# thetisproject/thetis

Hardware: AMD Instinct MI355X
Metric: DG element-updates/sec, 2D SWE DG-P1 SSPRK33 (higher is better)
Workload: dtype f64

## Files before the change

thetis_amd/csrc/swe2d_api_fuse.hip:

```cpp
#include "swe2d_handle.h"
#include "swe2d_fuse.h"
#include "swe2d_tiles.h"

#include <type_traits>

namespace swe2d_impl {

namespace {
template <bool... B, class F> auto pick_instance(F f) { return f(std::bool_constant<B>{}...); }
template <bool... B, class F, class... Rest> auto pick_instance(F f, bool b, Rest... rest)
{
    return b ? pick_instance<B..., true>(f, rest...) : pick_instance<B..., false>(f, rest...);
}

const TileSpec kPairTiles{3, 1, SWE_FUSE_WG, SWE_FUSE_INNER, SWE_FUSE_RING, SWE_FUSE_MAX_OUT, false};
const TileSpec kQuadPairTiles{4, 1, SWE_FUSE_WG, SWE_QFUSE_INNER, SWE_QFUSE_RING, SWE_QFUSE_MAX_OUT, false};
const TileSpec kTripleTiles{3, 2, SWE_FUSE_WG, SWE_FUSE_WG, -1, SWE_FUSE3_MAX_OUT, true, true};

int build_table(Handle *h, const TileSpec &spec, const std::vector<int> &order, const std::vector<unsigned char> &start, TileTable &t)
{
    const int n = h->n_cells;
    std::string err;
    if (build_tiles(h->h_nbr.data(), h->stride, n, (int)order.size() == n ? order.data() : nullptr,
                    (int)start.size() == n ? start.data() : nullptr, spec, t, err))
        return fail(h, SWE2D_ERR_UNSUPPORTED, err);
    return SWE2D_OK;
}

std::vector<int> tile_records(const TileTable &t, int nfacets)
{
    std::vector<int> rec;
    for (size_t i = 0; i < t.cell.size(); i++) {
        const unsigned *w = &t.facet[i*nfacets];
        rec.push_back(t.cell[i]);
        rec.push_back((int)(w[0] | (w[1] << SWE_FUSE_FBITS) | (w[2] << (2*SWE_FUSE_FBITS))));
        if (nfacets == 4) { rec.push_back((int)w[3]); rec.push_back(0); }
    }
    return rec;
}

int upload_tiles(Handle *h, TileSet &ts, const std::vector<int> &rec, const std::vector<int> &counts, const TileTable &t,
                 const std::vector<unsigned> *slot_data = nullptr)
{
    HIP_TRY(h, hipMalloc(&ts.tile, rec.size()*sizeof(int)));
    HIP_TRY(h, hipMalloc(&ts.counts, counts.size()*sizeof(int)));
    HIP_TRY(h, hipMemcpy(ts.tile, rec.data(), rec.size()*sizeof(int), hipMemcpyHostToDevice));
    HIP_TRY(h, hipMemcpy(ts.counts, counts.data(), counts.size()*sizeof(int), hipMemcpyHostToDevice));
    std::vector<int> slots;
    for (size_t i = 0; i + 1 < t.slot_first.size(); i++) { slots.push_back(t.slot_first[i]); slots.push_back(t.slot_first[i + 1] - t.slot_first[i]); }
    std::vector<int> src(t.slot_src);
    if (slot_data) src.assign(slot_data->begin(), slot_data->end());
    src.push_back(0);
    HIP_TRY(h, hipMalloc(&ts.slots, slots.size()*sizeof(int)));
    HIP_TRY(h, hipMalloc(&ts.slot_src, src.size()*sizeof(int)));
    HIP_TRY(h, hipMemcpy(ts.slots, slots.data(), slots.size()*sizeof(int), hipMemcpyHostToDevice));
    HIP_TRY(h, hipMemcpy(ts.slot_src, src.data(), src.size()*sizeof(int), hipMemcpyHostToDevice));
    ts.n_tiles = (int)t.n_inner.size();
    ts.ring[0] = t.ring[0]; ts.ring[1] = t.ring[1];
    return SWE2D_OK;
}
}

void free_tiles(TileSet &ts)
{
    if (ts.tile) (void)hipFree(ts.tile);
    if (ts.counts) (void)hipFree(ts.counts);
    if (ts.slots) (void)hipFree(ts.slots);
    if (ts.slot_src) (void)hipFree(ts.slot_src);
    ts = TileSet();
}

int fuse12_build(Handle *h)
{
    TileSet &ts = pair_tiles(h);
    if (ts.tile || h->fuse_state == -1 || stream_capturing(h)) return SWE2D_OK;
    TileTable t;
    if (int rc = build_table(h, h->npc == 4 ? kQuadPairTiles : kPairTiles, h->fuse_order, {}, t)) return rc;
    if (!fuse12_tiles_pay(h, (int)t.n_inner.size())) { h->fuse_state = -1; return SWE2D_OK; }
    return upload_tiles(h, ts, tile_records(t, h->npc), t.n_inner, t);
}

template <class Args>
static int launch_pair(Handle *h, void (*kern)(const Args), int cell_end)
{
    const TileSet &ts = pair_tiles(h);
    if (!ts.tile) return fail(h, SWE2D_ERR_UNSUPPORTED, "fused stage pair: no tile tables");
    Args q;
    fill_stage_args(h, q.st, 0, 0, 2, 0.0, 1.0, kBeta[0], 0, h->n_owned);
    q.st.idxc = h->opt[SWE2D_OPT_COMPACT_IDX] == 0 ? nullptr : h->idxc;
    q.tile = static_cast<decltype(q.tile)>(ts.tile);
    q.n_inner = ts.counts;
    q.n_tiles = ts.n_tiles;
    q.cell_end = cell_end;
    q.beta1 = kBeta[0];
    q.a0_2 = kAlpha0[1]; q.a1_2 = kAlphaIn[1]; q.beta2 = kBeta[1];
    q.out = h->state[2];
    const int grid = ((ts.n_tiles + 7)/8)*8;
    SWE_CHK_SYNC(h->stream);
    hipLaunchKernelGGL(kern, dim3(grid), dim3(SWE_FUSE_WG), 0, h->stream, q);
    HIP_TRY(h, hipGetLastError());
    stage_written(h, false, true);
    return SWE2D_OK;
}

int launch_fuse12(Handle *h, int cell_end)
{
    const bool nl = h->par.use_nonlinear_equations != 0, lf = h->par.use_lax_friedrichs_velocity != 0;
    if (h->npc == 4)
        return launch_pair(h, pick_instance([](auto a, auto b, auto c, auto d) -> void (*)(const SweFuseQuadArgs) {
                               return swe_fuse12_quad_kernel<a.value, b.value, c.value, d.value>; }, nl, lf, has_sources(h), h->affine), cell_end);
    return launch_pair(h, pick_instance([](auto a, auto b, auto c) -> void (*)(const SweFuseArgs) {
                           return swe_fuse12_kernel<a.value, b.value, c.value>; }, nl, lf, has_sources(h)), cell_end);
}

int fuse123_build(Handle *h)
{
    if (h->fuse3.tile || stream_capturing(h)) return SWE2D_OK;
    TileTable t;
    if (int rc = build_table(h, kTripleTiles, (int)h->fuse3_order.size() == h->n_cells ? h->fuse3_order : h->fuse_order, h->fuse3_start, t)) return rc;
    std::vector<int> counts;
    for (size_t i = 0; i < t.n_inner.size(); i++) { counts.push_back(t.n_inner[i]); counts.push_back(t.n_mid[i] | (t.rot[i] << 16)); }
    LaneRecords r;
    build_lane_records(t, h->h_nbr.data(), h->h_cv.data(), h->stride, SWE_FUSE_WG, 8u*SWE_FUSE3_XG, (unsigned)h->stride*8u, r);
    return upload_tiles(h, h->fuse3, r.lane, counts, t, &r.slot);
}

int launch_fuse123(Handle *h, int cell_end)
{
    if (int rc = capture_parity_check(h)) return rc;
    if (int rc = fuse123_build(h)) return rc;
    if (!h->fuse3.tile) return fail(h, SWE2D_ERR_UNSUPPORTED, "fused stages: no tile tables (not built inside a stream capture)");
    SweFuse3Args q;
    fill_stage_args(h, q.st, 0, 0, 1, 0.0, 1.0, kBeta[0], 0, h->n_owned);
    q.rec = static_cast<const int4 *>(h->fuse3.tile);
    q.counts = reinterpret_cast<const int2 *>(h->fuse3.counts);
    q.slots = reinterpret_cast<const int2 *>(h->fuse3.slots);
    q.slot_off = reinterpret_cast<const uint2 *>(h->fuse3.slot_src);
    q.n_tiles = h->fuse3.n_tiles;
    q.cell_end = cell_end;
    for (int s = 0; s < 3; s++) { q.a0[s] = s ? kAlpha0[s] : 0.0; q.a1[s] = s ? kAlphaIn[s] : 1.0; q.beta[s] = kBeta[s]; }
    q.out = h->state[1];
    auto kern = pick_instance([](auto a, auto b, auto c) -> void (*)(const SweFuse3Args) { return swe_fuse123_kernel<a.value, b.value, c.value>; },
                              h->par.use_nonlinear_equations != 0, h->par.use_lax_friedrichs_velocity != 0, has_sources(h));
    const int grid = ((h->fuse3.n_tiles + 7)/8)*8;
    SWE_CHK_SYNC(h->stream);
    hipLaunchKernelGGL(kern, dim3(grid), dim3(SWE_FUSE_WG), 0, h->stream, q);
    HIP_TRY(h, hipGetLastError());
    swap_state_buffers(h);
    unsigned long long id = 0;
    if (stream_capturing(h, &id)) {
        if (id != h->capture_id) { h->capture_id = id; h->capture_swaps = 0; }
        h->capture_swaps++;
    }
    return SWE2D_OK;
}

int capture_parity_check(Handle *h)
{
    if (h->capture_swaps == 0 && h->capture_odd == 0) return SWE2D_OK;
    unsigned long long id = 0;
    const bool capturing = stream_capturing(h, &id);
    if (h->capture_swaps) {
        if (capturing && id == h->capture_id) return SWE2D_OK;
        if (h->capture_swaps & 1) { swap_state_buffers(h); h->capture_odd++; }
        h->capture_swaps = 0;
    }
    if (capturing || h->capture_odd == 0) return SWE2D_OK;
    const int odd = h->capture_odd;
    h->capture_odd = 0;
    return fail(h, SWE2D_ERR_UNSUPPORTED, std::to_string(odd) + " stream capture(s) recorded an odd number of swe2d_solve_step_cells launches: "
                "such a graph ends on the other state buffer than it began on and cannot be replayed (the state is the one from before the "
                "capture); capture an even number per sequence");
}

}

static int checked_tile_order(Handle *h, const int32_t *cells, std::vector<int> &order)
{
    std::vector<char> seen((size_t)h->n_cells, 0);
    for (int i = 0; cells && i < h->n_cells; i++) {
        if (cells[i] < 0 || cells[i] >= h->n_cells || seen[cells[i]]) return fail(h, SWE2D_ERR_INVALID_ARGUMENT, "fused stages: the tile order is not a permutation of the cells");
        seen[cells[i]] = 1;
    }
    if (cells) order.assign(cells, cells + h->n_cells);
    return SWE2D_OK;
}

extern "C" {

int swe2d_fused_set_order(swe2d_handle *hh, const int32_t *cells_in_tile_order)
{
    Handle *h = H(hh);
    if (!h) return SWE2D_ERR_INVALID_ARGUMENT;
    HIP_TRY(h, hipSetDevice(h->device));
    std::vector<int> order;
    if (int rc = checked_tile_order(h, cells_in_tile_order, order)) return rc;
    HIP_TRY(h, hipStreamSynchronize(h->stream));
    for (TileSet *ts : {&h->fuse, &h->fuseq, &h->fuse3}) free_tiles(*ts);
    if (h->fuse_state == -1) h->fuse_state = 0;
    h->fuse_order.swap(order);
    return SWE2D_OK;
}

int swe2d_fused_set_triple_tiles(swe2d_handle *hh, const int32_t *cells_in_tile_order, const int32_t *tile_starts, int32_t n_starts)
{
    Handle *h = H(hh);
    if (!h) return SWE2D_ERR_INVALID_ARGUMENT;
    HIP_TRY(h, hipSetDevice(h->device));
    std::vector<int> order;
    std::vector<unsigned char> start;
    if (int rc = checked_tile_order(h, cells_in_tile_order, order)) return rc;
    if (n_starts < 0 || (n_starts > 0 && !tile_starts)) return fail(h, SWE2D_ERR_INVALID_ARGUMENT, "fused stages: tile starts");
    if (n_starts > 0) {
        start.assign((size_t)h->n_cells, 0);
        for (int i = 0; i < n_starts; i++) {
            if (tile_starts[i] < 0 || tile_starts[i] >= h->n_cells) return fail(h, SWE2D_ERR_INVALID_ARGUMENT, "fused stages: a tile start outside the cells");
            start[tile_starts[i]] = 1;
        }
    }
    HIP_TRY(h, hipStreamSynchronize(h->stream));
    free_tiles(h->fuse3);
    h->fuse3_order.swap(order);
    h->fuse3_start.swap(start);
    return SWE2D_OK;
}

static int fused_triple_info(Handle *h, StepCaller who, int32_t out[4])
{
    if (!h || !out) return fail(h, SWE2D_ERR_INVALID_ARGUMENT, "null argument");
    out[0] = out[1] = out[2] = out[3] = 0;
    HIP_TRY(h, hipSetDevice(h->device));
    StepPath path;
    if (int rc = step_ready(h, who, kTriple, &path)) return rc;
    if (path != kTriple) return SWE2D_OK;
    out[0] = 1; out[1] = h->fuse3.n_tiles; out[2] = (int32_t)h->fuse3.ring[0]; out[3] = (int32_t)h->fuse3.ring[1];
    return SWE2D_OK;
}
int swe2d_fused_triple_info(swe2d_handle *hh, int32_t out[4]) { return fused_triple_info(H(hh), kWholeStep, out); }
int swe2d_fused_step_info(swe2d_handle *hh, int32_t out[4]) { return fused_triple_info(H(hh), kPartitionStep, out); }

int swe2d_solve_step_cells(swe2d_handle *hh, int32_t cell_end)
{
    Handle *h = H(hh);
    if (!h) return SWE2D_ERR_INVALID_ARGUMENT;
    if (cell_end < 0 || cell_end > h->n_cells) return fail(h, SWE2D_ERR_INVALID_ARGUMENT, "bad cell range");
    if (!(step_kernels(h) & kTriple)) return fail(h, SWE2D_ERR_UNSUPPORTED, "swe2d_solve_step_cells: the three-stage kernel does not cover this handle");
    HIP_TRY(h, hipSetDevice(h->device));
    if (int rc = capture_parity_check(h)) return rc;
    if (!h->fuse3.tile && stream_capturing(h))
        return fail(h, SWE2D_ERR_UNSUPPORTED, "swe2d_solve_step_cells: first call inside a stream capture (swe2d_fused_step_info builds the tables)");
    return launch_fuse123(h, cell_end);
}

int swe2d_solve_stage_pair_cells(swe2d_handle *hh, int32_t cell_end_0, int32_t cell_end_1)
{
    Handle *h = H(hh);
    if (!h) return SWE2D_ERR_INVALID_ARGUMENT;
    if (cell_end_1 < 0 || cell_end_1 > cell_end_0 || cell_end_0 > h->n_cells) return fail(h, SWE2D_ERR_INVALID_ARGUMENT, "bad cell ranges");
    if (forced(h)) return fail(h, SWE2D_ERR_UNSUPPORTED, "swe2d_solve_stage_pair_cells: not with a tide table or an atmospheric record (swe2d_tide_eval / swe2d_atm_eval + swe2d_solve_stage_cells per stage)");
    HIP_TRY(h, hipSetDevice(h->device));
    if (int rc = capture_parity_check(h)) return rc;
    StepPath path;
    if (int rc = step_ready(h, kPartitionPair, kPair, &path)) return rc;
    if (path == kPair) return launch_fuse12(h, cell_end_1);
    if (int rc = stage_on_range(h, 0, 0, cell_end_0)) return rc;
    return stage_on_range(h, 1, 0, cell_end_1);
}

}
```

thetis_amd/csrc/swe2d_fuse.h:

```cpp
#pragma once
#include "swe2d_kernels.h"
#include "swe2d_flow.h"

#ifndef SWE_FUSE_WG
#define SWE_FUSE_WG 256
#endif
#ifndef SWE_FUSE_MIN_WG
#define SWE_FUSE_MIN_WG 3
#endif
#ifndef SWE_FUSE_INNER
#define SWE_FUSE_INNER 192
#endif
#define SWE_FUSE_FBITS 10
#define SWE_FUSE_RING (SWE_FUSE_WG - SWE_FUSE_INNER)
#define SWE_FUSE_XG (9*SWE_FUSE_WG)
#define SWE_FUSE_MAX_OUT (2*SWE_FUSE_RING)
#define SWE_FUSE_LDS (SWE_FUSE_XG + 6*SWE_FUSE_MAX_OUT)

struct SweFuseArgs {
    SweStageArgs st;
    const int2 *tile;
    const int *n_inner;
    int n_tiles;
    int cell_end;
// ... 68 lines not shown
            py[i] = swe_ld(rvy, v8, 0);
            h[i] = swe_ld(rvh, v8, 0);
        }
#pragma unroll
        for (int f = 0; f < 3; f++) {
            const int b = (f + 1) % 3;
            nx[f] = py[b] - py[f];
            ny[f] = px[f] - px[b];
        }
#pragma unroll
        for (int i = 0; i < 3; i++) { lds[i*SWE_FUSE_WG + lane] = u[i]; lds[(3 + i)*SWE_FUSE_WG + lane] = v[i]; lds[(6 + i)*SWE_FUSE_WG + lane] = e[i]; }
#pragma unroll
        for (int f = 0; f < 3; f++) {
            if (outside[f]) {
                const unsigned at = ((unsigned)tl.y >> (SWE_FUSE_FBITS*f)) & 0x1ffu;
#pragma unroll
                for (int j = 0; j < 6; j++) lds[SWE_LDSI(SWE_FUSE_XG + 6*at + j, SWE_FUSE_LDS)] = r0[f][j];
            }
        }
    }
    __syncthreads();
    double o1u[3], o1v[3], o1e[3];
    double twoA = 0.0;
    if (real) {
        twoA = fma(nx[0], ny[1], -(ny[0]*nx[1]));
        double bu[3], bv[3], be[3], wu[3], wv[3], we[3];
        double H[3];
        swe_tri_depths<NONLIN, false>(h, e, nullptr, H);
        swe_tri_cell<NONLIN>(p.g, u, v, e, H, nx, ny, bu, bv, be);
        swe_flow_rhs_facets<NONLIN, LF, SRC, 1, false, SWE_FUSE_XG, SWE_FUSE_WG, SWE_FUSE_LDS>(p, k, u, v, e, h, lds, tr, bmarkers, nx, ny, twoA, bu, bv, be);
#pragma unroll
        for (int i = 0; i < 3; i++) { wu[i] = 1.0*u[i]; wv[i] = 1.0*v[i]; we[i] = 1.0*e[i]; }
        swe_tri_finish<NONLIN, LF, false, true>(p, k, q.beta1, twoA, u, v, e, h, nullptr, nullptr, nx, ny, bmarkers, bkind1, bu, bv, be,
                                                wu, wv, we, true, o1u, o1v, o1e);
    }
    __syncthreads();
    if (real) {
#pragma unroll
        for (int i = 0; i < 3; i++) { lds[i*SWE_FUSE_WG + lane] = o1u[i]; lds[(3 + i)*SWE_FUSE_WG + lane] = o1v[i]; lds[(6 + i)*SWE_FUSE_WG + lane] = o1e[i]; }
    }
    const bool act2 = lane < n_inner && k < q.cell_end;
    if (act2) {
#pragma unroll
        for (int i = 0; i < 3; i++) {
            lw[i][lane] = fma(q.a0_2, u[i], q.a1_2*o1u[i]);
            lw[3 + i][lane] = fma(q.a0_2, v[i], q.a1_2*o1v[i]);
            lw[6 + i][lane] = fma(q.a0_2, e[i], q.a1_2*o1e[i]);
        }
    }
    __syncthreads();
    if (act2) {
#pragma unroll
        for (int i = 0; i < 3; i++) asm volatile("" : "+v"(nx[i]), "+v"(ny[i]), "+v"(h[i]));
#pragma unroll
        for (int f = 0; f < 3; f++) asm volatile("" : "+v"(tr[f][0]));
        asm volatile("" : "+v"(bmarkers), "+v"(twoA));
        double bu[3], bv[3], be[3], wu[3], wv[3], we[3], ou[3], ov[3], oe[3];
        double H[3];
        swe_tri_depths<NONLIN, false>(h, o1e, nullptr, H);
        swe_tri_cell<NONLIN>(p.g, o1u, o1v, o1e, H, nx, ny, bu, bv, be);
        swe_flow_rhs_facets<NONLIN, LF, SRC, 1, false, SWE_FUSE_XG, SWE_FUSE_WG, SWE_FUSE_LDS>(p, k, o1u, o1v, o1e, h, lds, tr, bmarkers, nx, ny, twoA, bu, bv, be);
#pragma unroll
        for (int i = 0; i < 3; i++) { wu[i] = lw[i][lane]; wv[i] = lw[3 + i][lane]; we[i] = lw[6 + i][lane]; }
        swe_tri_finish<NONLIN, LF, false, true>(p, k, q.beta2, twoA, o1u, o1v, o1e, h, nullptr, nullptr, nx, ny, bmarkers, bkind1, bu, bv, be,
                                                wu, wv, we, true, ou, ov, oe);
        const swe_rsrc_t gou = swe_rsrc(q.out), gov = swe_rsrc(q.out + 3*S), goe = swe_rsrc(q.out + 6*S);
#pragma unroll
        for (int i = 0; i < 3; i++) {
            swe_st(gou, k8, i*S8, ou[i]);
            swe_st(gov, k8, i*S8, ov[i]);
            swe_st(goe, k8, i*S8, oe[i]);
        }
    }
}

#ifndef SWE_FUSE3_MAX_OUT
#define SWE_FUSE3_MAX_OUT 224
#endif
#ifndef SWE_FUSE3_GEOM
#define SWE_FUSE3_GEOM 1
#endif
#define SWE_FUSE3_NGEO 7
#define SWE_FUSE3_GEO (18*SWE_FUSE_WG)
#define SWE_FUSE3_XG (SWE_FUSE3_GEOM ? 9*SWE_FUSE_WG : 18*SWE_FUSE_WG)
#define SWE_FUSE3_LDS (SWE_FUSE3_GEOM ? SWE_FUSE3_GEO + SWE_FUSE3_NGEO*SWE_FUSE_WG : SWE_FUSE3_XG + 6*SWE_FUSE3_MAX_OUT)
static_assert(6*SWE_FUSE3_MAX_OUT <= 9*SWE_FUSE_WG, "the staging area must fit P1");
#ifndef SWE_FUSE3_SRC_MIN_WG
#define SWE_FUSE3_SRC_MIN_WG 2
#endif

struct SweFuse3Args {
    SweStageArgs st;
    const int4 *rec;
    const int2 *counts;
    const int2 *slots;
    const uint2 *slot_off;
    int n_tiles;
    int cell_end;
    double a0[3], a1[3], beta[3];
    double *out;
};

template <bool NONLIN, bool LF, bool SRC = false>
__global__ __launch_bounds__(SWE_FUSE_WG, SRC ? SWE_FUSE3_SRC_MIN_WG : SWE_FUSE_MIN_WG) void swe_fuse123_kernel(const SweFuse3Args q)
{
#pragma clang fp contract(off)
    __shared__ double lds[SWE_FUSE3_LDS];
    const SweStageArgs &p = q.st;
    const int tile = swe_logical_block(blockIdx.x, gridDim.x);
    if (tile >= q.n_tiles) return;
    const int lane = (int)threadIdx.x;
    const int4 *const rec = q.rec + (size_t)tile*(2*SWE_FUSE_WG) + lane;
    const int4 ra = rec[0];
    const int4 rb = rec[SWE_FUSE_WG];
    const bool real = ra.x >= 0;
    const int k = real ? ra.x : 0;
    const int2 cnt = q.counts[tile];
    const int n_inner = cnt.x, n_mid = cnt.y & 0xffff, rot64 = (cnt.y >> 16) << 6;
    const size_t S = p.stride;
    const unsigned S8 = (unsigned)S*8u, k8 = (unsigned)k*8u;
    double *const P1 = lds + 9*SWE_FUSE_WG;
#ifdef SWE_WAVE_TIMING
    int wt_bodies = __any(real) ? 1 : 0;
#endif
    const int2 sl = q.slots[tile];
    const int slot = ((lane & 63) << 2) | (lane >> 6);
    const bool has_slot = slot < sl.y;
    uint2 so = {0u, 0u};
    if (has_slot) so = q.slot_off[sl.x + slot];

    int bmarkers = rb.w, bkind1 = 0;
    unsigned tr[3][1] = {{(unsigned)ra.y}, {(unsigned)ra.z}, {(unsigned)ra.w}};
    double h[3], nx[3], ny[3], u[3], v[3], e[3];
    double px[3], py[3];
    const swe_rsrc_t gu = swe_rsrc(p.uin), gv = swe_rsrc(p.uin + 3*S), ge = swe_rsrc(p.uin + 6*S);
    if (real) {
        if (bmarkers != 0) {
            const int m1 = (bmarkers & 0xff) ? (bmarkers & 0xff) : ((bmarkers & 0xff00) ? ((bmarkers >> 8) & 0xff) : (bmarkers >> 16));
            bkind1 = m1 < SWE_MAX_MARKERS ? p.bc.kind[m1] : 0;
        }
#pragma unroll
        for (int i = 0; i < 3; i++) {
            u[i] = swe_ld(gu, k8, i*S8);
            v[i] = swe_ld(gv, k8, i*S8);
            e[i] = swe_ld(ge, k8, i*S8);
        }
        const swe_rsrc_t rvx = swe_rsrc(p.vx), rvy = swe_rsrc(p.vy), rvh = swe_rsrc(p.vh);
        const unsigned v8[3] = {(unsigned)rb.x, (unsigned)rb.y, (unsigned)rb.z};
#pragma unroll
        for (int i = 0; i < 3; i++) {
            px[i] = swe_ld(rvx, v8[i], 0);
            py[i] = swe_ld(rvy, v8[i], 0);
            h[i] = swe_ld(rvh, v8[i], 0);
        }
    }
    double r0[6];
    if (has_slot) {
        const unsigned ob = so.x, oa = so.y;
        r0[0] = swe_ld(gu, ob, 0); r0[1] = swe_ld(gv, ob, 0); r0[2] = swe_ld(ge, ob, 0);
        r0[3] = swe_ld(gu, oa, 0); r0[4] = swe_ld(gv, oa, 0); r0[5] = swe_ld(ge, oa, 0);
    }
    if (real) {
#pragma unroll
        for (int f = 0; f < 3; f++) {
            const int b = (f + 1) % 3;
            nx[f] = py[b] - py[f];
            ny[f] = px[f] - px[b];
        }
#pragma unroll
        for (int i = 0; i < 3; i++) { lds[i*SWE_FUSE_WG + lane] = u[i]; lds[(3 + i)*SWE_FUSE_WG + lane] = v[i]; lds[(6 + i)*SWE_FUSE_WG + lane] = e[i]; }
    }
    if (has_slot) {
#pragma unroll
        for (int j = 0; j < 6; j++) lds[SWE_LDSI(SWE_FUSE3_XG + 6*slot + j, SWE_FUSE3_LDS)] = r0[j];
    }
    __syncthreads();
    constexpr int GEOM1 = SWE_FUSE3_GEOM ? SWE_GEOM_KEEP : SWE_GEOM_COMPUTE, GEOM23 = SWE_FUSE3_GEOM ? SWE_GEOM_STORED : SWE_GEOM_COMPUTE;
    double twoA = 0.0;
    double *const G = lds + SWE_FUSE3_GEO + lane;
    if (real) {
        twoA = fma(nx[0], ny[1], -(ny[0]*nx[1]));
        double bu[3], bv[3], be[3], wu[3], wv[3], we[3], ou[3], ov[3], oe[3];
        double H[3];
        swe_tri_depths<NONLIN, false>(h, e, nullptr, H);
        swe_tri_cell<NONLIN>(p.g, u, v, e, H, nx, ny, bu, bv, be);
        swe_flow_rhs_facets<NONLIN, LF, SRC, 1, false, SWE_FUSE3_XG, SWE_FUSE_WG, SWE_FUSE3_LDS, GEOM1, SWE_TR_BYTES, true>(p, k, u, v, e, h, lds, tr, bmarkers, nx, ny, twoA, bu, bv, be,
                                                                                                     nullptr, nullptr, G);
#pragma unroll
        for (int i = 0; i < 3; i++) { wu[i] = 1.0*u[i]; wv[i] = 1.0*v[i]; we[i] = 1.0*e[i]; }
        swe_tri_finish<NONLIN, LF, false, true, GEOM1, SWE_FUSE_WG>(p, k, q.beta[0], twoA, u, v, e, h, nullptr, nullptr, nx, ny, bmarkers, bkind1,
                                                                    bu, bv, be, wu, wv, we, true, ou, ov, oe, G);
#pragma unroll
        for (int i = 0; i < 3; i++) { u[i] = ou[i]; v[i] = ov[i]; e[i] = oe[i]; }
    }
    if (SWE_FUSE3_GEOM) __syncthreads();
    if (real) {
#pragma unroll
        for (int i = 0; i < 3; i++) { P1[i*SWE_FUSE_WG + lane] = u[i]; P1[(3 + i)*SWE_FUSE_WG + lane] = v[i]; P1[(6 + i)*SWE_FUSE_WG + lane] = e[i]; }
    }
    __syncthreads();
#pragma unroll 1
    for (int s = 1; s < 3; s++) {
        const int role = (lane - rot64) & (SWE_FUSE_WG - 1);
        const bool act = role < (s == 1 ? n_mid : n_inner) && (s == 1 || k < q.cell_end);
#ifdef SWE_WAVE_TIMING
        wt_bodies += __any(act) ? 1 : 0;
#endif
        double ou[3], ov[3], oe[3];
        if (act) {
#pragma unroll
            for (int i = 0; i < 3; i++) asm volatile("" : "+v"(nx[i]), "+v"(ny[i]), "+v"(h[i]));
#pragma unroll
            for (int f = 0; f < 3; f++) asm volatile("" : "+v"(tr[f][0]));
            asm volatile("" : "+v"(bmarkers));
            if (SRC || !SWE_FUSE3_GEOM) asm volatile("" : "+v"(twoA));
            double bu[3], bv[3], be[3], wu[3], wv[3], we[3];
            double H[3];
            swe_tri_depths<NONLIN, false>(h, e, nullptr, H);
            swe_tri_cell<NONLIN>(p.g, u, v, e, H, nx, ny, bu, bv, be);
            swe_flow_rhs_facets<NONLIN, LF, SRC, 1, false, SWE_FUSE3_XG, SWE_FUSE_WG, 9*SWE_FUSE_WG, GEOM23, SWE_TR_BYTES_INSIDE, true>(p, k, u, v, e, h, P1, tr, bmarkers, nx, ny, twoA, bu, bv, be,
                                                                                                          nullptr, nullptr, G);
            const double a0 = q.a0[s], a1 = q.a1[s];
#pragma unroll
            for (int i = 0; i < 3; i++) {
                wu[i] = fma(a0, lds[i*SWE_FUSE_WG + lane], a1*u[i]);
                wv[i] = fma(a0, lds[(3 + i)*SWE_FUSE_WG + lane], a1*v[i]);
                we[i] = fma(a0, lds[(6 + i)*SWE_FUSE_WG + lane], a1*e[i]);
            }
            swe_tri_finish<NONLIN, LF, false, true, GEOM23, SWE_FUSE_WG>(p, k, q.beta[s], twoA, u, v, e, h, nullptr, nullptr, nx, ny, bmarkers,
                                                                         bkind1, bu, bv, be, wu, wv, we, true, ou, ov, oe, G);
        }
        if (s == 1) {
            __syncthreads();
            if (act) {
#pragma unroll
                for (int i = 0; i < 3; i++) { P1[i*SWE_FUSE_WG + lane] = ou[i]; P1[(3 + i)*SWE_FUSE_WG + lane] = ov[i]; P1[(6 + i)*SWE_FUSE_WG + lane] = oe[i]; }
#pragma unroll
                for (int i = 0; i < 3; i++) { u[i] = ou[i]; v[i] = ov[i]; e[i] = oe[i]; }
            }
            __syncthreads();
        } else if (act) {
            const swe_rsrc_t gou = swe_rsrc(q.out), gov = swe_rsrc(q.out + 3*S), goe = swe_rsrc(q.out + 6*S);
#pragma unroll
            for (int i = 0; i < 3; i++) {
                swe_st(gou, k8, i*S8, ou[i]);
                swe_st(gov, k8, i*S8, ov[i]);
                swe_st(goe, k8, i*S8, oe[i]);
            }
        }
    }
#ifdef SWE_WAVE_TIMING
    if ((lane & 63) == 0 && 4*blockIdx.x + (lane >> 6) < 6*SWE_WT_MAX) {
        unsigned hw, xcc;
        asm volatile("s_getreg_b32 %0, hwreg(HW_REG_HW_ID)" : "=s"(hw));
        asm volatile("s_getreg_b32 %0, hwreg(HW_REG_XCC_ID)" : "=s"(xcc));
        (&swe_wave_ts[0][0])[4*blockIdx.x + (lane >> 6)] = (unsigned long long)hw | ((unsigned long long)(xcc & 0xf) << 32)
                                                           | ((unsigned long long)wt_bodies << 40) | (1ull << 44);
    }
#endif
}


#define SWE_QFUSE_INNER 192
#define SWE_QFUSE_RING (SWE_FUSE_WG - SWE_QFUSE_INNER)
#define SWE_QFUSE_XG (12*SWE_FUSE_WG)
#define SWE_QFUSE_MAX_OUT (3*SWE_QFUSE_RING)
#define SWE_QFUSE_LDS (SWE_QFUSE_XG + 6*SWE_QFUSE_MAX_OUT)

struct SweFuseQuadArgs {
    SweStageArgs st;
    const int4 *tile;
    const int *n_inner;
    int n_tiles;
    int cell_end;
    double beta1, a0_2, a1_2, beta2;
    double *out;
};

template <bool NONLIN, bool LF, bool SRC, bool AFFINE>
__global__ __launch_bounds__(SWE_FUSE_WG, SWE_FUSE_MIN_WG) void swe_fuse12_quad_kernel(const SweFuseQuadArgs q)
{
#pragma clang fp contract(off)
    __shared__ double lds[SWE_QFUSE_LDS];
    __shared__ double lu0[12*SWE_QFUSE_INNER];
    const SweStageArgs &p = q.st;
    const int tile = swe_logical_block(blockIdx.x, gridDim.x);
    if (tile >= q.n_tiles) return;
    const int lane = (int)threadIdx.x;
    const int4 tl = q.tile[(size_t)tile*SWE_FUSE_WG + lane];
    const bool real = tl.x >= 0;
    const int k = real ? tl.x : 0;
    const int n_inner = q.n_inner[tile];
    const size_t S = p.stride;
    const unsigned S8 = (unsigned)S*8u, k8 = (unsigned)k*8u, S4 = (unsigned)S*4u, k4 = (unsigned)k*4u;

    unsigned tr[4] = {0u, 0u, 0u, 0u}, bmarkers = 0u;
    int nb[4] = {-1, -1, -1, -1}, vid[4] = {0, 0, 0, 0};
    double u[4], v[4], e[4];
    if (real) {
#pragma unroll
        for (int i = 0; i < 4; i++) {
            nb[i] = swe_ldi(swe_rsrc(p.nbr), k4, i*S4);
            vid[i] = swe_ldi(swe_rsrc(p.cv), k4, i*S4);
        }
        const swe_rsrc_t gu = swe_rsrc(p.uin), gv = swe_rsrc(p.uin + 4*S), ge = swe_rsrc(p.uin + 8*S);
#pragma unroll
        for (int i = 0; i < 4; i++) {
            u[i] = swe_ld(gu, k8, i*S8);
            v[i] = swe_ld(gv, k8, i*S8);
            e[i] = swe_ld(ge, k8, i*S8);
        }
        bmarkers = (nb[0] < 0 ? (unsigned)(-nb[0]) : 0u) | (nb[1] < 0 ? (unsigned)(-nb[1]) << 8 : 0u) |
                   (nb[2] < 0 ? (unsigned)(-nb[2]) << 16 : 0u) | (nb[3] < 0 ? (unsigned)(-nb[3]) << 24 : 0u);
        double r0[4][6];
        bool outside[4];
#pragma unroll
        for (int f = 0; f < 4; f++) {
            const int nbf = nb[f];
            const unsigned w = f < 3 ? (((unsigned)tl.y >> (SWE_FUSE_FBITS*f)) & 0x3ffu) : ((unsigned)tl.z & 0x3ffu);
            outside[f] = (w & 0x200u) != 0u;
            const unsigned at = w & 0x1ffu;
            const int f2 = nbf >= 0 ? (nbf & 3) : f, na = (f2 + 1) & 3;
            const unsigned ab = outside[f] ? (unsigned)(SWE_QFUSE_XG + 6*at) : (unsigned)(f2*SWE_FUSE_WG + at);
            const unsigned aa = outside[f] ? (unsigned)(SWE_QFUSE_XG + 6*at + 3) : (unsigned)(na*SWE_FUSE_WG + at);
            tr[f] = ab | (aa << 16);
            const int code = outside[f] ? nbf : ((k << 2) | f);
            const unsigned kn8 = (unsigned)(code >> 2)*8u;
            const int g2 = code & 3, ga = (g2 + 1) & 3;
            const unsigned ob = kn8 + ((g2 & 1) ? S8 : 0u) + ((g2 & 2) ? 2u*S8 : 0u);
            const unsigned oa = kn8 + ((ga & 1) ? S8 : 0u) + ((ga & 2) ? 2u*S8 : 0u);
            r0[f][0] = swe_ld(gu, ob, 0); r0[f][1] = swe_ld(gv, ob, 0); r0[f][2] = swe_ld(ge, ob, 0);
            r0[f][3] = swe_ld(gu, oa, 0); r0[f][4] = swe_ld(gv, oa, 0); r0[f][5] = swe_ld(ge, oa, 0);
        }
#pragma unroll
        for (int i = 0; i < 4; i++) { lds[i*SWE_FUSE_WG + lane] = u[i]; lds[(4 + i)*SWE_FUSE_WG + lane] = v[i]; lds[(8 + i)*SWE_FUSE_WG + lane] = e[i]; }
#pragma unroll
        for (int f = 0; f < 4; f++) {
            if (outside[f]) {
                const unsigned at = (f < 3 ? ((unsigned)tl.y >> (SWE_FUSE_FBITS*f)) : (unsigned)tl.z) & 0x1ffu;
#pragma unroll
// ... 50 lines not shown
```

thetis_amd/csrc/swe2d_handle.h:

```cpp
#pragma once
#include "../../include/swe2d.h"
#include "swe2d_kernels.h"
#include "swe2d_sipg.h"
#include "swe2d_flow.h"
#include "swe2d_p2p.h"

#include <dlfcn.h>
#include <unistd.h>

#include <algorithm>
#include <cmath>
#include <cstdio>
#include <cstdlib>
#include <cstring>
#include <new>
#include <string>
#include <vector>
#include <atomic>
#include <mutex>

static_assert(SWE2D_MAX_MARKERS == SWE_MAX_MARKERS, "marker table size mismatch");
static_assert(SWE2D_MAX_FARMS == SWE_MAX_FARMS && SWE2D_MAX_THRUST_TABLE == SWE_MAX_THRUST_TABLE, "turbine farm table size mismatch");

#ifdef SWE_RANGE_CHECK
#include <map>
#include <mutex>
namespace {
std::mutex g_chk_mutex;
std::map<unsigned long long, unsigned long long> g_chk_allocs;
bool g_chk_dirty = true;
unsigned long long g_chk_launches = 0;
void swe_chk_upload_locked()
{
    static SweChkTable t;
    t.n = 0;
    for (auto &kv : g_chk_allocs) if (t.n < SWE_CHK_MAX) { t.lo[t.n] = kv.first; t.hi[t.n] = kv.second; t.n++; }
    (void)hipDeviceSynchronize();
    (void)hipMemcpyToSymbol(HIP_SYMBOL(swe_chk_tab), &t, sizeof(t));
    g_chk_dirty = false;
}
hipError_t swe_chk_malloc(void **p, size_t n)
{
    const hipError_t e = hipMalloc(p, n);
    if (e == hipSuccess && *p) {
        std::lock_guard<std::mutex> lock(g_chk_mutex);
        const char *st = getenv("THETIS_AMD_RANGE_SELFTEST");
        g_chk_allocs[(unsigned long long)*p] = (unsigned long long)*p + ((st && atoi(st)) ? n/2 : n);
        swe_chk_upload_locked();
    }
    return e;
}
template <class T> hipError_t swe_chk_malloc(T **p, size_t n) { return swe_chk_malloc((void **)p, n); }
hipError_t swe_chk_free(void *p)
{
    { std::lock_guard<std::mutex> lock(g_chk_mutex); g_chk_allocs.erase((unsigned long long)p); g_chk_dirty = true; }
    return hipFree(p);
}
void swe_chk_sync(hipStream_t stream)
{
    std::lock_guard<std::mutex> lock(g_chk_mutex);
    g_chk_launches++;
    if (!g_chk_dirty) return;
    hipStreamCaptureStatus cs = hipStreamCaptureStatusNone;
    if (stream && hipStreamIsCapturing(stream, &cs) == hipSuccess && cs != hipStreamCaptureStatusNone) return;
    swe_chk_upload_locked();
}
}
#define hipMalloc(p, n) swe_chk_malloc(p, n)
#define hipFree(p) swe_chk_free(p)
#define SWE_CHK_SYNC(stream) swe_chk_sync(stream)
extern "C" int swe2d_debug_range_report(unsigned long long out[5])
{
    std::lock_guard<std::mutex> lock(g_chk_mutex);
    (void)hipDeviceSynchronize();
    if (hipMemcpyFromSymbol(out, HIP_SYMBOL(swe_chk_report), 4*sizeof(unsigned long long)) != hipSuccess) return 1;
    out[3] = g_chk_launches;
    out[4] = g_chk_allocs.size();
    return 0;
}
#else
#define SWE_CHK_SYNC(stream) ((void)0)
#endif

namespace swe2d_impl {

extern thread_local std::string g_create_error;

extern const double kBeta[3], kAlpha0[3], kAlphaIn[3];

extern std::atomic<unsigned long long> g_next_uid;

struct TileSet {
    void *tile = nullptr;
    int *counts = nullptr;
    int *slots = nullptr;
    int *slot_src = nullptr;
    int n_tiles = 0;
    long long ring[2] = {0, 0};
};

struct Handle {
    unsigned long long uid = g_next_uid.fetch_add(1ull);
    int device = 0;
    hipStream_t stream = nullptr;
    bool own_stream = false;
    hipStream_t my_stream = nullptr;
    hipStream_t xstream = nullptr;
    int n_cells = 0, n_owned = 0, n_interior = 0, n_vertices = 0;
    int npc = 3;
    bool affine = true;
    bool affine_local = true;
    size_t stride = 0;
    double *state[3] = {nullptr, nullptr, nullptr};
    int *nbr = nullptr, *cv = nullptr;
    struct FacetList { std::vector<int32_t> cells, facets; int *dev = nullptr; };
    FacetList facet_lists[8];
    int facet_list_next = 0;
    int4 *opp4 = nullptr;
    int *bnd_cells = nullptr;
    int n_bnd = 0;
    int opt[SWE2D_OPT_COUNT];
    Handle() { for (int i = 0; i < SWE2D_OPT_COUNT; i++) opt[i] = -1; }
    bool stage_valid[2] = {false, false};
    int capture_swaps = 0;
    unsigned long long capture_id = 0;
    int capture_odd = 0;
    int4 *idx4 = nullptr;
    int2 *idx2 = nullptr;
    int4 *idxc = nullptr;
    TileSet fuse, fuseq, fuse3;
    int fuse_state = 0;
    std::vector<int> fuse_order;
    std::vector<int> fuse3_order;
    std::vector<unsigned char> fuse3_start;
    int n_conn_escapes = 0;
    std::vector<int> h_nbr;
    std::vector<int> h_cv;
    unsigned *flow_flag = nullptr, *flow_status = nullptr;
    int4 *flow_xo4 = nullptr;
    int2 *flow_xo2 = nullptr;
    int2 *flow_xblk = nullptr;
    int *flow_xsrc = nullptr;
    std::vector<int> h_send, h_recv;
    std::vector<int> flow_fpos;
    int2 *flow_xsend = nullptr;
    int *flow_xrecv = nullptr;
    unsigned *flow_xtick = nullptr;
    int flow_push_blocks = 0, flow_recv_blocks = 0;
    bool flow_x_ready = false;
    int *flow_cell = nullptr;
    unsigned flow_parity_bytes = 0;
    void *flow_ex = nullptr;
    size_t flow_ex_bytes = 0;
    int flow_blocks = 0;
    int flow_capacity = -1;
    int flow_max_rim = 0;
    int launch_parity = 0;
    bool flow_used = false;
    double *vx = nullptr, *vy = nullptr, *vh = nullptr;
    double *bc_field[4] = {nullptr, nullptr, nullptr, nullptr};
    double *valpha = nullptr;
    bool wd = false;
    bool state_holds_D = false;
    struct Snapshot { void *data = nullptr; size_t bytes = 0; bool holds_D = false; };
    Snapshot snapshot[SWE2D_SNAPSHOT_SLOTS];
    bool visc = false;
    double *nu_v = nullptr;
    double nu_const = 0.0, sipg_factor = 1.0;
    int visc_grad_div = 0, visc_grad_depth = 1;
    double *field[SWE2D_FIELD_COUNT] = {nullptr, nullptr, nullptr, nullptr, nullptr, nullptr, nullptr, nullptr, nullptr};
    double scalar[SWE2D_SCALAR_COUNT] = {-1.0, -1.0, -1.0, 0.0, -1.0};
    double *stage_uv = nullptr, *stage_eta = nullptr;
    double *partial = nullptr;
    int n_partial_blocks = 0;
    unsigned long long *diag_acc = nullptr;
    int *send_cells = nullptr, *recv_cells = nullptr;
    int n_send = 0, n_recv = 0;
    struct P2p {
        void *zone = nullptr;
// ... 293 lines not shown
```

thetis_amd/csrc/swe2d_tiles.h:

```cpp
#pragma once
#include <algorithm>
#include <cstddef>
#include <string>
#include <utility>
#include <vector>

#ifndef SWE_FUSE3_ROT
#define SWE_FUSE3_ROT(tile) ((int)(((unsigned)(tile)*0x9E3779B1u) >> 30))
#endif

namespace swe2d_impl {

constexpr unsigned kTileOutside = 0x200u;

struct TileSpec {
    int nfacets;
    int rings;
    int wg;
    int max_inner;
    int max_ring1;
    int max_out;
    bool rotate;
    bool group_walls = false;
};
// ... 82 lines not shown
                std::vector<int> cand[3];
                for (int cls = 0; cls < 3; cls++) {
                    const int w = (int)walls[cls].size(), room = (int)rest[cls].size();
                    cand[cls].push_back(cls == 0 ? room : 0);
                    cand[cls].push_back(cls == 0 ? 0 : room);
                    for (int edge = 64; edge < wg && w > 0; edge += 64)
                        for (int o : {edge - bound[cls], edge - w - bound[cls]}) if (o > 0 && o < room) cand[cls].push_back(o);
                }
                for (int o0 : cand[0]) for (int o1 : cand[1]) for (int o2 : cand[2]) {
                    const int off[3] = {o0, o1, o2};
                    std::fill(mark.begin(), mark.end(), 0);
                    for (int cls = 0; cls < 3; cls++)
                        for (int l = 0; l < (int)walls[cls].size(); l++) mark[bound[cls] + off[cls] + l] = 1;
                    const int pairs = pairs_of(mark.data());
                    if (pairs < best) { best = pairs; best_off[0] = o0; best_off[1] = o1; best_off[2] = o2; }
                }
                if (best_off[0] >= 0) {
                    std::vector<int> sorted;
                    for (int cls = 0; cls < 3; cls++) {
                        sorted.insert(sorted.end(), rest[cls].begin(), rest[cls].begin() + best_off[cls]);
                        sorted.insert(sorted.end(), walls[cls].begin(), walls[cls].end());
                        sorted.insert(sorted.end(), rest[cls].begin() + best_off[cls], rest[cls].end());
                    }
                    cells.swap(sorted);
                }
            }
        }
        if (nt != count[1] + count[2] + count[3] || ni != count[1] || nt > wg) { err = std::string(who) + "tile bookkeeping"; return 1; }
        const int tile = (int)t.n_inner.size();
        const int rot = sp.rotate ? SWE_FUSE3_ROT(tile) & 3 : 0;
        auto phys = [rot, wg](int role) { return (role + 64*rot) & (wg - 1); };
        for (int l = 0; l < nt; l++) lane_of[cells[l]] = phys(l);
        const size_t base = (size_t)tile*wg;
        t.cell.resize(base + wg, -1);
        t.facet.resize((base + wg)*nf, 0u);
        const int outermost = sp.rings == 2 ? nm : ni;
        int n_out = 0;
        for (int l = 0; l < nt; l++) {
            const int c = cells[l];
            t.cell[base + phys(l)] = c;
            for (int f = 0; f < nf; f++) {
                const int code = nbr[(size_t)f*stride + c];
                unsigned field;
                if (code < 0) field = (unsigned)phys(l);
                else if (state[code >> 2] != 0) field = (unsigned)lane_of[code >> 2];
                else {
                    if (l < outermost || n_out >= sp.max_out) { err = std::string(who) + "ring bookkeeping"; return 1; }
                    field = kTileOutside | (unsigned)n_out++;
                    t.slot_src.push_back(code);
                }
                t.facet[(base + phys(l))*nf + f] = field;
            }
        }
        t.n_inner.push_back(ni); t.n_mid.push_back(nm); t.rot.push_back(rot);
        t.ring[0] += count[2]; t.ring[1] += count[3];
        t.slot_first.push_back((int)t.slot_src.size());
        for (int c : cells) { state[c] = 0; lane_of[c] = -1; }
    }
    return 0;
}

inline long long wall_wave_stages(const TileTable &t, const int *nbr, size_t stride, int nfacets, int wg, int tile = -1)
{
    long long pairs = 0;
    const int n_tiles = (int)t.n_inner.size();
    for (int tl = tile < 0 ? 0 : tile; tl < (tile < 0 ? n_tiles : tile + 1); tl++) {
        unsigned waves[3] = {0u, 0u, 0u};
        for (int l = 0; l < wg; l++) {
            const int c = t.cell[(size_t)tl*wg + l];
            if (c < 0) continue;
            bool wall = false;
            for (int f = 0; f < nfacets; f++) wall = wall || nbr[(size_t)f*stride + c] < 0;
            if (!wall) continue;
            const int role = (l - 64*t.rot[tl]) & (wg - 1);
            waves[0] |= 1u << (l >> 6);
            if (role < t.n_mid[tl]) waves[1] |= 1u << (l >> 6);
            if (role < t.n_inner[tl]) waves[2] |= 1u << (l >> 6);
        }
        for (int s = 0; s < 3; s++) for (unsigned w = waves[s]; w; w &= w - 1) pairs++;
    }
    return pairs;
}

struct LaneRecords {
    std::vector<int> lane;
    std::vector<unsigned> slot;
};

inline void build_lane_records(const TileTable &t, const int *nbr, const int *cv, size_t stride, int wg, unsigned xg_bytes, unsigned s8,
                               LaneRecords &r)
{
    const size_t n_tiles = t.n_inner.size();
    r.lane.assign(n_tiles*2*(size_t)wg*4, 0);
    r.slot.assign(2*t.slot_src.size(), 0u);
    const unsigned plane = 8u*(unsigned)wg;
    for (size_t tile = 0; tile < n_tiles; tile++) {
        for (int l = 0; l < wg; l++) {
            int *a = &r.lane[((2*tile + 0)*wg + l)*4], *b = &r.lane[((2*tile + 1)*wg + l)*4];
            const int c = t.cell[tile*wg + l];
            a[0] = c;
            if (c < 0) { a[0] = -1; continue; }
            unsigned bm = 0u;
            for (int f = 0; f < 3; f++) {
                const int code = nbr[(size_t)f*stride + c];
                const unsigned w = t.facet[(tile*wg + l)*3 + f], at = w & 0x1ffu;
                const unsigned g = code >= 0 ? (unsigned)(code & 3) : (unsigned)f, ga = g == 2u ? 0u : g + 1u;
                const bool outside = (w & kTileOutside) != 0u;
                const unsigned ab = outside ? xg_bytes + 48u*at : plane*g + 8u*at;
                const unsigned aa = outside ? xg_bytes + 24u + 48u*at : plane*ga + 8u*at;
                a[1 + f] = (int)(ab | (aa << 16));
                if (code < 0) bm |= (unsigned)(-code) << (8*f);
                b[f] = (int)((unsigned)cv[(size_t)f*stride + c]*8u);
            }
            b[3] = (int)bm;
        }
    }
    for (size_t s = 0; s < t.slot_src.size(); s++) {
        const unsigned code = (unsigned)t.slot_src[s], kn8 = (code >> 2)*8u, g = code & 3u;
        r.slot[2*s] = kn8 + (g == 0u ? 0u : (g == 1u ? s8 : 2u*s8));
        r.slot[2*s + 1] = kn8 + (g == 0u ? s8 : (g == 1u ? 2u*s8 : 0u));
    }
}

}
```

Measured before the change: 34.70 billion.

## Stage halo slots in per-lane LDS planes with per-lane slot offset table

Replaces the per-tile slot list (slots + slot_src indirection) with a precomputed per-lane slot offset table, so each lane loads its staging offsets with one coalesced read instead of a dependent two-level lookup. Halo values are now staged in LDS as component planes indexed by lane instead of 6-double interleaved slots, and the facet address records are rewritten to match. This aims to remove the dependent global load and LDS bank conflicts from strided slot writes and reads, at the cost of a larger per-lane table and a slightly different LDS footprint. It also adds optional wave-timing instrumentation behind a compile flag.

```diff
diff --git a/thetis_amd/csrc/swe2d_api_fuse.hip b/thetis_amd/csrc/swe2d_api_fuse.hip
--- a/thetis_amd/csrc/swe2d_api_fuse.hip
+++ b/thetis_amd/csrc/swe2d_api_fuse.hip
@@ -40,21 +40,16 @@
 }
 
 int upload_tiles(Handle *h, TileSet &ts, const std::vector<int> &rec, const std::vector<int> &counts, const TileTable &t,
-                 const std::vector<unsigned> *slot_data = nullptr)
+                 const std::vector<unsigned> *lane_slot = nullptr)
 {
     HIP_TRY(h, hipMalloc(&ts.tile, rec.size()*sizeof(int)));
     HIP_TRY(h, hipMalloc(&ts.counts, counts.size()*sizeof(int)));
     HIP_TRY(h, hipMemcpy(ts.tile, rec.data(), rec.size()*sizeof(int), hipMemcpyHostToDevice));
     HIP_TRY(h, hipMemcpy(ts.counts, counts.data(), counts.size()*sizeof(int), hipMemcpyHostToDevice));
-    std::vector<int> slots;
-    for (size_t i = 0; i + 1 < t.slot_first.size(); i++) { slots.push_back(t.slot_first[i]); slots.push_back(t.slot_first[i + 1] - t.slot_first[i]); }
-    std::vector<int> src(t.slot_src);
-    if (slot_data) src.assign(slot_data->begin(), slot_data->end());
-    src.push_back(0);
-    HIP_TRY(h, hipMalloc(&ts.slots, slots.size()*sizeof(int)));
-    HIP_TRY(h, hipMalloc(&ts.slot_src, src.size()*sizeof(int)));
-    HIP_TRY(h, hipMemcpy(ts.slots, slots.data(), slots.size()*sizeof(int), hipMemcpyHostToDevice));
-    HIP_TRY(h, hipMemcpy(ts.slot_src, src.data(), src.size()*sizeof(int), hipMemcpyHostToDevice));
+    if (lane_slot) {
+        HIP_TRY(h, hipMalloc(&ts.lane_slot, lane_slot->size()*sizeof(unsigned)));
+        HIP_TRY(h, hipMemcpy(ts.lane_slot, lane_slot->data(), lane_slot->size()*sizeof(unsigned), hipMemcpyHostToDevice));
+    }
     ts.n_tiles = (int)t.n_inner.size();
     ts.ring[0] = t.ring[0]; ts.ring[1] = t.ring[1];
     return SWE2D_OK;
@@ -65,8 +60,7 @@
 {
     if (ts.tile) (void)hipFree(ts.tile);
     if (ts.counts) (void)hipFree(ts.counts);
-    if (ts.slots) (void)hipFree(ts.slots);
-    if (ts.slot_src) (void)hipFree(ts.slot_src);
+    if (ts.lane_slot) (void)hipFree(ts.lane_slot);
     ts = TileSet();
 }
 
@@ -121,8 +115,9 @@
     std::vector<int> counts;
     for (size_t i = 0; i < t.n_inner.size(); i++) { counts.push_back(t.n_inner[i]); counts.push_back(t.n_mid[i] | (t.rot[i] << 16)); }
     LaneRecords r;
-    build_lane_records(t, h->h_nbr.data(), h->h_cv.data(), h->stride, SWE_FUSE_WG, 8u*SWE_FUSE3_XG, (unsigned)h->stride*8u, r);
-    return upload_tiles(h, h->fuse3, r.lane, counts, t, &r.slot);
+    build_lane_records(t, h->h_nbr.data(), h->h_cv.data(), h->stride, SWE_FUSE_WG, 8u*SWE_FUSE3_XG, (unsigned)h->stride*8u, r,
+                       SWE_FUSE3_STAGING_PLANES ? kStagingPlanes : kStagingSlot6);
+    return upload_tiles(h, h->fuse3, r.lane, counts, t, &r.lane_slot);
 }
 
 int launch_fuse123(Handle *h, int cell_end)
@@ -134,8 +129,7 @@
     fill_stage_args(h, q.st, 0, 0, 1, 0.0, 1.0, kBeta[0], 0, h->n_owned);
     q.rec = static_cast<const int4 *>(h->fuse3.tile);
     q.counts = reinterpret_cast<const int2 *>(h->fuse3.counts);
-    q.slots = reinterpret_cast<const int2 *>(h->fuse3.slots);
-    q.slot_off = reinterpret_cast<const uint2 *>(h->fuse3.slot_src);
+    q.lane_slot = reinterpret_cast<const uint2 *>(h->fuse3.lane_slot);
     q.n_tiles = h->fuse3.n_tiles;
     q.cell_end = cell_end;
     for (int s = 0; s < 3; s++) { q.a0[s] = s ? kAlpha0[s] : 0.0; q.a1[s] = s ? kAlphaIn[s] : 1.0; q.beta[s] = kBeta[s]; }
@@ -267,4 +261,16 @@
     return stage_on_range(h, 1, 0, cell_end_1);
 }
 
-}
+#ifdef SWE_WAVE_TIMING
+int swe2d_debug_read_fuse3_phases(swe2d_handle *hh, unsigned long long *out, int32_t n_wg, int32_t info[3])
+{
+    Handle *h = H(hh);
+    if (!h || !info || n_wg < 0 || n_wg > SWE_F3P_MAX_WG) return SWE2D_ERR_INVALID_ARGUMENT;
+    info[0] = SWE_F3P_WORDS; info[1] = SWE_F3P_STAMPS; info[2] = SWE_F3P_MAX_WG;
+    HIP_TRY(h, hipStreamSynchronize(h->stream));
+    if (n_wg > 0) HIP_TRY(h, hipMemcpyFromSymbol(out, HIP_SYMBOL(swe_fuse3_phase), sizeof(unsigned long long)*4*SWE_F3P_WORDS*(size_t)n_wg));
+    return SWE2D_OK;
+}
+#endif
+
+}
diff --git a/thetis_amd/csrc/swe2d_fuse.h b/thetis_amd/csrc/swe2d_fuse.h
--- a/thetis_amd/csrc/swe2d_fuse.h
+++ b/thetis_amd/csrc/swe2d_fuse.h
@@ -174,9 +174,14 @@
 #endif
 #define SWE_FUSE3_NGEO 7
 #define SWE_FUSE3_GEO (18*SWE_FUSE_WG)
+#ifndef SWE_FUSE3_STAGING_PLANES
+#define SWE_FUSE3_STAGING_PLANES 1
+#endif
 #define SWE_FUSE3_XG (SWE_FUSE3_GEOM ? 9*SWE_FUSE_WG : 18*SWE_FUSE_WG)
-#define SWE_FUSE3_LDS (SWE_FUSE3_GEOM ? SWE_FUSE3_GEO + SWE_FUSE3_NGEO*SWE_FUSE_WG : SWE_FUSE3_XG + 6*SWE_FUSE3_MAX_OUT)
-static_assert(6*SWE_FUSE3_MAX_OUT <= 9*SWE_FUSE_WG, "the staging area must fit P1");
+#define SWE_FUSE3_XG_DOUBLES (SWE_FUSE3_STAGING_PLANES ? 8*SWE_FUSE_WG : 6*SWE_FUSE3_MAX_OUT)
+#define SWE_FUSE3_LDS (SWE_FUSE3_GEOM ? SWE_FUSE3_GEO + SWE_FUSE3_NGEO*SWE_FUSE_WG : SWE_FUSE3_XG + SWE_FUSE3_XG_DOUBLES)
+static_assert(SWE_FUSE3_XG_DOUBLES <= 9*SWE_FUSE_WG, "the staging area must fit P1");
+static_assert(SWE_FUSE3_MAX_OUT <= 4*(SWE_FUSE_WG/4 - 1) + 4 && SWE_FUSE3_MAX_OUT <= SWE_FUSE_WG, "a lane per staging slot");
 #ifndef SWE_FUSE3_SRC_MIN_WG
 #define SWE_FUSE3_SRC_MIN_WG 2
 #endif
@@ -185,19 +190,34 @@
     SweStageArgs st;
     const int4 *rec;
     const int2 *counts;
-    const int2 *slots;
-    const uint2 *slot_off;
+    const uint2 *lane_slot;
     int n_tiles;
     int cell_end;
     double a0[3], a1[3], beta[3];
     double *out;
 };
 
+#ifdef SWE_WAVE_TIMING
+#define SWE_F3P_STAMPS 13
+#define SWE_F3P_WORDS 16
+#define SWE_F3P_MAX_WG 8192
+__device__ unsigned long long swe_fuse3_phase[SWE_F3P_MAX_WG][4][SWE_F3P_WORDS];
+#define SWE_F3T(i, ...) asm volatile("s_memtime %0\n\ts_waitcnt lgkmcnt(0)" : "=s"(wt[i]) : __VA_ARGS__ : "memory")
+#define SWE_F3T9(i, a, b, c) SWE_F3T(i, "v"(a[0]), "v"(a[1]), "v"(a[2]), "v"(b[0]), "v"(b[1]), "v"(b[2]), "v"(c[0]), "v"(c[1]), "v"(c[2]))
+#else
+#define SWE_F3T(i, ...)
+#define SWE_F3T9(i, a, b, c)
+#endif
+
 template <bool NONLIN, bool LF, bool SRC = false>
 __global__ __launch_bounds__(SWE_FUSE_WG, SRC ? SWE_FUSE3_SRC_MIN_WG : SWE_FUSE_MIN_WG) void swe_fuse123_kernel(const SweFuse3Args q)
 {
 #pragma clang fp contract(off)
     __shared__ double lds[SWE_FUSE3_LDS];
+#ifdef SWE_WAVE_TIMING
+    unsigned long long wt[SWE_F3P_STAMPS] = {};
+    SWE_F3T(0, "s"(0));
+#endif
     const SweStageArgs &p = q.st;
     const int tile = swe_logical_block(blockIdx.x, gridDim.x);
     if (tile >= q.n_tiles) return;
@@ -215,11 +235,9 @@
 #ifdef SWE_WAVE_TIMING
     int wt_bodies = __any(real) ? 1 : 0;
 #endif
-    const int2 sl = q.slots[tile];
-    const int slot = ((lane & 63) << 2) | (lane >> 6);
-    const bool has_slot = slot < sl.y;
-    uint2 so = {0u, 0u};
-    if (has_slot) so = q.slot_off[sl.x + slot];
+    const uint2 so = q.lane_slot[(size_t)tile*SWE_FUSE_WG + lane];
+    const bool has_slot = so.x != 0xffffffffu;
+    SWE_F3T(1, "v"(ra.x), "v"(rb.x), "v"(so.x));
 
     int bmarkers = rb.w, bkind1 = 0;
     unsigned tr[3][1] = {{(unsigned)ra.y}, {(unsigned)ra.z}, {(unsigned)ra.w}};
@@ -253,6 +271,10 @@
         r0[3] = swe_ld(gu, oa, 0); r0[4] = swe_ld(gv, oa, 0); r0[5] = swe_ld(ge, oa, 0);
     }
     if (real) {
+#ifdef SWE_WAVE_TIMING
+        SWE_F3T9(2, px, py, h);
+        SWE_F3T9(2, u, v, e);
+#endif
 #pragma unroll
         for (int f = 0; f < 3; f++) {
             const int b = (f + 1) % 3;
@@ -263,11 +285,23 @@
         for (int i = 0; i < 3; i++) { lds[i*SWE_FUSE_WG + lane] = u[i]; lds[(3 + i)*SWE_FUSE_WG + lane] = v[i]; lds[(6 + i)*SWE_FUSE_WG + lane] = e[i]; }
     }
     if (has_slot) {
+        SWE_F3T(3, "v"(r0[0]), "v"(r0[1]), "v"(r0[2]), "v"(r0[3]), "v"(r0[4]), "v"(r0[5]));
+#if SWE_FUSE3_STAGING_PLANES
+#pragma unroll
+        for (int c = 0; c < 3; c++) {
+            lds[SWE_LDSI(SWE_FUSE3_XG + 3*c*SWE_FUSE_WG + lane, SWE_FUSE3_LDS)] = r0[c];
+            lds[SWE_LDSI(SWE_FUSE3_XG + (3*c + 1)*SWE_FUSE_WG + lane, SWE_FUSE3_LDS)] = r0[3 + c];
+        }
+#else
+        const int slot = ((lane & 63) << 2) | (lane >> 6);
 #pragma unroll
         for (int j = 0; j < 6; j++) lds[SWE_LDSI(SWE_FUSE3_XG + 6*slot + j, SWE_FUSE3_LDS)] = r0[j];
-    }
-    __syncthreads();
+#endif
+    }
+    __syncthreads();
+    SWE_F3T(4, "s"(0));
     constexpr int GEOM1 = SWE_FUSE3_GEOM ? SWE_GEOM_KEEP : SWE_GEOM_COMPUTE, GEOM23 = SWE_FUSE3_GEOM ? SWE_GEOM_STORED : SWE_GEOM_COMPUTE;
+    constexpr int TRB1 = SWE_FUSE3_STAGING_PLANES ? SWE_TR_BYTES_INSIDE : SWE_TR_BYTES;
     double twoA = 0.0;
     double *const G = lds + SWE_FUSE3_GEO + lane;
     if (real) {
@@ -276,7 +310,7 @@
         double H[3];
         swe_tri_depths<NONLIN, false>(h, e, nullptr, H);
         swe_tri_cell<NONLIN>(p.g, u, v, e, H, nx, ny, bu, bv, be);
-        swe_flow_rhs_facets<NONLIN, LF, SRC, 1, false, SWE_FUSE3_XG, SWE_FUSE_WG, SWE_FUSE3_LDS, GEOM1, SWE_TR_BYTES, true>(p, k, u, v, e, h, lds, tr, bmarkers, nx, ny, twoA, bu, bv, be,
+        swe_flow_rhs_facets<NONLIN, LF, SRC, 1, false, SWE_FUSE3_XG, SWE_FUSE_WG, SWE_FUSE3_LDS, GEOM1, TRB1, true>(p, k, u, v, e, h, lds, tr, bmarkers, nx, ny, twoA, bu, bv, be,
                                                                                                      nullptr, nullptr, G);
 #pragma unroll
         for (int i = 0; i < 3; i++) { wu[i] = 1.0*u[i]; wv[i] = 1.0*v[i]; we[i] = 1.0*e[i]; }
@@ -284,15 +318,17 @@
                                                                     bu, bv, be, wu, wv, we, true, ou, ov, oe, G);
 #pragma unroll
         for (int i = 0; i < 3; i++) { u[i] = ou[i]; v[i] = ov[i]; e[i] = oe[i]; }
+        SWE_F3T9(5, u, v, e);
     }
     if (SWE_FUSE3_GEOM) __syncthreads();
+    SWE_F3T(6, "s"(0));
     if (real) {
 #pragma unroll
         for (int i = 0; i < 3; i++) { P1[i*SWE_FUSE_WG + lane] = u[i]; P1[(3 + i)*SWE_FUSE_WG + lane] = v[i]; P1[(6 + i)*SWE_FUSE_WG + lane] = e[i]; }
     }
     __syncthreads();
-#pragma unroll 1
-    for (int s = 1; s < 3; s++) {
+    SWE_F3T(7, "s"(0));
+    auto later_stage = [&](const int s) __attribute__((always_inline)) {
         const int role = (lane - rot64) & (SWE_FUSE_WG - 1);
         const bool act = role < (s == 1 ? n_mid : n_inner) && (s == 1 || k < q.cell_end);
 #ifdef SWE_WAVE_TIMING
@@ -321,9 +357,13 @@
             }
             swe_tri_finish<NONLIN, LF, false, true, GEOM23, SWE_FUSE_WG>(p, k, q.beta[s], twoA, u, v, e, h, nullptr, nullptr, nx, ny, bmarkers,
                                                                          bkind1, bu, bv, be, wu, wv, we, true, ou, ov, oe, G);
+#ifdef SWE_WAVE_TIMING
+            if (s == 1) SWE_F3T9(8, ou, ov, oe); else SWE_F3T9(11, ou, ov, oe);
+#endif
         }
         if (s == 1) {
             __syncthreads();
+            SWE_F3T(9, "s"(0));
             if (act) {
 #pragma unroll
                 for (int i = 0; i < 3; i++) { P1[i*SWE_FUSE_WG + lane] = ou[i]; P1[(3 + i)*SWE_FUSE_WG + lane] = ov[i]; P1[(6 + i)*SWE_FUSE_WG + lane] = oe[i]; }
@@ -331,6 +371,7 @@
                 for (int i = 0; i < 3; i++) { u[i] = ou[i]; v[i] = ov[i]; e[i] = oe[i]; }
             }
             __syncthreads();
+            SWE_F3T(10, "s"(0));
         } else if (act) {
             const swe_rsrc_t gou = swe_rsrc(q.out), gov = swe_rsrc(q.out + 3*S), goe = swe_rsrc(q.out + 6*S);
 #pragma unroll
@@ -340,7 +381,9 @@
                 swe_st(goe, k8, i*S8, oe[i]);
             }
         }
-    }
+    };
+    later_stage(1);
+    later_stage(2);
 #ifdef SWE_WAVE_TIMING
     if ((lane & 63) == 0 && 4*blockIdx.x + (lane >> 6) < 6*SWE_WT_MAX) {
         unsigned hw, xcc;
@@ -348,6 +391,20 @@
         asm volatile("s_getreg_b32 %0, hwreg(HW_REG_XCC_ID)" : "=s"(xcc));
         (&swe_wave_ts[0][0])[4*blockIdx.x + (lane >> 6)] = (unsigned long long)hw | ((unsigned long long)(xcc & 0xf) << 32)
                                                            | ((unsigned long long)wt_bodies << 40) | (1ull << 44);
+    }
+    asm volatile("s_waitcnt vmcnt(0)" ::: "memory");
+    SWE_F3T(12, "s"(0));
+    const unsigned wt_every = (gridDim.x + SWE_F3P_MAX_WG - 1)/SWE_F3P_MAX_WG;
+    if ((lane & 63) == 0 && blockIdx.x % wt_every == 0) {
+        unsigned hw, xcc;
+        asm volatile("s_getreg_b32 %0, hwreg(HW_REG_HW_ID)" : "=s"(hw));
+        asm volatile("s_getreg_b32 %0, hwreg(HW_REG_XCC_ID)" : "=s"(xcc));
+        unsigned long long *const w = swe_fuse3_phase[blockIdx.x/wt_every][lane >> 6];
+#pragma unroll
+        for (int i = 0; i < SWE_F3P_STAMPS; i++) w[i] = wt[i];
+        w[13] = (unsigned long long)tile;
+        w[14] = (unsigned long long)hw | ((unsigned long long)(xcc & 0xf) << 32) | ((unsigned long long)wt_bodies << 40) | (1ull << 44);
+        w[15] = 0ull;
     }
 #endif
 }
diff --git a/thetis_amd/csrc/swe2d_handle.h b/thetis_amd/csrc/swe2d_handle.h
--- a/thetis_amd/csrc/swe2d_handle.h
+++ b/thetis_amd/csrc/swe2d_handle.h
@@ -93,8 +93,7 @@
 struct TileSet {
     void *tile = nullptr;
     int *counts = nullptr;
-    int *slots = nullptr;
-    int *slot_src = nullptr;
+    unsigned *lane_slot = nullptr;
     int n_tiles = 0;
     long long ring[2] = {0, 0};
 };
diff --git a/thetis_amd/csrc/swe2d_tiles.h b/thetis_amd/csrc/swe2d_tiles.h
--- a/thetis_amd/csrc/swe2d_tiles.h
+++ b/thetis_amd/csrc/swe2d_tiles.h
@@ -188,17 +188,23 @@
     return pairs;
 }
 
+constexpr unsigned kNoSlot = 0xffffffffu;
+enum StagingLayout { kStagingSlot6 = 0, kStagingPlanes = 1 };
+inline unsigned lane_of_slot(unsigned s, int wg) { return (unsigned)(wg/4)*(s & 3u) + (s >> 2); }
+
 struct LaneRecords {
     std::vector<int> lane;
     std::vector<unsigned> slot;
+    std::vector<unsigned> lane_slot;
 };
 
 inline void build_lane_records(const TileTable &t, const int *nbr, const int *cv, size_t stride, int wg, unsigned xg_bytes, unsigned s8,
-                               LaneRecords &r)
+                               LaneRecords &r, StagingLayout staging = kStagingSlot6)
 {
     const size_t n_tiles = t.n_inner.size();
     r.lane.assign(n_tiles*2*(size_t)wg*4, 0);
     r.slot.assign(2*t.slot_src.size(), 0u);
+    r.lane_slot.assign(n_tiles*(size_t)wg*2, kNoSlot);
     const unsigned plane = 8u*(unsigned)wg;
     for (size_t tile = 0; tile < n_tiles; tile++) {
         for (int l = 0; l < wg; l++) {
@@ -212,8 +218,9 @@
                 const unsigned w = t.facet[(tile*wg + l)*3 + f], at = w & 0x1ffu;
                 const unsigned g = code >= 0 ? (unsigned)(code & 3) : (unsigned)f, ga = g == 2u ? 0u : g + 1u;
                 const bool outside = (w & kTileOutside) != 0u;
-                const unsigned ab = outside ? xg_bytes + 48u*at : plane*g + 8u*at;
-                const unsigned aa = outside ? xg_bytes + 24u + 48u*at : plane*ga + 8u*at;
+                unsigned ab = outside ? xg_bytes + 48u*at : plane*g + 8u*at;
+                unsigned aa = outside ? xg_bytes + 24u + 48u*at : plane*ga + 8u*at;
+                if (outside && staging == kStagingPlanes) { ab = xg_bytes + 8u*lane_of_slot(at, wg); aa = ab + plane; }
                 a[1 + f] = (int)(ab | (aa << 16));
                 if (code < 0) bm |= (unsigned)(-code) << (8*f);
                 b[f] = (int)((unsigned)cv[(size_t)f*stride + c]*8u);
@@ -226,6 +233,11 @@
         r.slot[2*s] = kn8 + (g == 0u ? 0u : (g == 1u ? s8 : 2u*s8));
         r.slot[2*s + 1] = kn8 + (g == 0u ? s8 : (g == 1u ? 2u*s8 : 0u));
     }
-}
-
-}
+    for (size_t tile = 0; tile < n_tiles; tile++)
+        for (int s = t.slot_first[tile]; s < t.slot_first[tile + 1]; s++) {
+            unsigned *ls = &r.lane_slot[(tile*wg + lane_of_slot((unsigned)(s - t.slot_first[tile]), wg))*2];
+            ls[0] = r.slot[2*(size_t)s]; ls[1] = r.slot[2*(size_t)s + 1];
+        }
+}
+
+}
```

Result: faster. 35.34 billion (median of 6 runs) (+1.8%).
